# algbio/SBWT

Hardware: AMD Instinct MI355X
Metric: k-mers/sec (whole node), plain-matrix k=30 streaming search (higher is better)
Workload: dtype u64

## Files before the change

sbwt_amd/csrc/sbwt_device.h:

```cpp
#pragma once
#include <stdint.h>

#define SBWT_MEGA_SHIFT 31
#define SBWT_GROUP_BASES 32

#ifndef SBWT_FUSED_SORT_DEFAULT
#define SBWT_FUSED_SORT_DEFAULT 3632
#endif
struct SbwtIndexView {
    const uint4 *blocks;
    const longlong2 *ptab;
    const unsigned long long *mega;
    long long n_nodes;
    long long n_pos;
    long long C[4];
    int k;
    int p_dev;
    int n_mega;
    int has_ssup;
    int probe_len;
    const uint4 *stab;
    int p_sparse;
    unsigned n_sb;
    const unsigned *col, *pos;
// ... 52 lines not shown
#define SBWT_SP_OVERFLOW (1ull << 62)
#define SBWT_SP_UNIQ 0x80000000u
#define SBWT_SP_MAX_DEPTH 31
#define SBWT_SP_HASH 0x9E3779B97F4A7C15ull
static __host__ __device__ inline unsigned long long sp2_hash(unsigned origin, unsigned long long key2) {
    unsigned long long h = (key2 ^ ((unsigned long long)origin << 17)) * SBWT_SP_HASH;
    h ^= h >> 31;
    return (h + origin) * 0xD6E8FEB86659FD93ull;
}
#define SBWT_SP2_USED 0x80000000u
#define SBWT_SP2_OVERFLOW 0x80000000u
static __host__ __device__ inline unsigned long long sbwt_pf_hash(unsigned long long key) { return key * SBWT_SP_HASH; }
static __host__ __device__ inline unsigned sbwt_pf_bits(unsigned long long h) { return (unsigned)(h >> 24) ^ (unsigned)(h >> 41); }

struct SbwtWorkHeader {
    unsigned long long ticket;
    int status;
    int rg_sample;
    unsigned long long n_stream;
    unsigned long long n_search;
    unsigned long long n_lf;
    unsigned long long n_tab_hit;
    unsigned long long n_ext;
    unsigned long long n_bridge;
    unsigned long long u_bad;
    long long u_read0, u_len, u_out0, u_stride;
    unsigned long long n_deferred;
    unsigned long long ticket2;
    unsigned long long n_pieces;
    unsigned long long pad[15];
    unsigned long long rg_long;
    unsigned long long n_ftick;
    unsigned long long ftick_over;
    unsigned long long pad2[5];
    unsigned long long hint;
};
#define SBWT_WS_CLEAR_BYTES (sizeof(SbwtWorkHeader) - 8)

#define SBWT_PIECE 1024
struct SbwtPieceTab {
    uint4 *pairs = nullptr;
    uint4 *outs = nullptr;
    long long cap = 0;
    int piece = SBWT_PIECE;
};
static_assert(sizeof(SbwtWorkHeader) == 320, "workspace header is 320 bytes");
struct SbwtTickTab {
    uint4 *tick = nullptr;
    unsigned *tick_read = nullptr;
    unsigned *defer_bits = nullptr;
    long long cap = 0;
};
#define SBWT_HINT_MAGIC 0x5B377A00u
#define SBWT_HINT_RATIO 12
#define SBWT_HINT_CALLS 2

void sbwt_launch_encode(const char *d_bases, long long total_bases, uint4 *d_packed, SbwtWorkHeader *ws,
                        hipStream_t stream);
void sbwt_launch_search(const SbwtIndexView &ix, const uint4 *d_packed, const long long *d_read_off,
                        const long long *d_out_off, long long *d_out, long long n_reads, SbwtWorkHeader *ws,
                        int streaming, hipStream_t stream, int variant, long long total_groups, void *d_sort_scratch,
                        long long sort_scratch_bytes, int sort_key_bits, SbwtPieceTab pt);
void sbwt_launch_search_fused(const SbwtIndexView &ix, const char *d_bases, long long total_bases, uint4 *d_packed,
                              const long long *d_read_off, const long long *d_out_off, long long *d_out, long long n_reads,
                              SbwtWorkHeader *ws, int streaming, hipStream_t stream, unsigned *d_defer,
                              hipEvent_t ev_begin, hipEvent_t ev_end, SbwtPieceTab pt, int ragged_ok, SbwtTickTab tt = SbwtTickTab());
void sbwt_launch_encode_chained(const char *d_bases, long long total_bases, uint4 *d_packed, SbwtWorkHeader *ws,
// ... 64 lines not shown
```

sbwt_amd/csrc/sbwt_kernels_common.h:

```cpp
#pragma once
#include <hip/hip_runtime.h>
#include <cstdio>
#include <cstdlib>
#include "sbwt_device.h"

typedef unsigned long long u64;
typedef long long i64;

#define SBWT_ERR_NOT_SINGLETON (-7)
#define SBWT_ERR_STALLED (-10)

__device__ __forceinline__ unsigned dna_code(unsigned b) { return ((b >> 1) & 3u) ^ ((b >> 2) & 1u); }
__device__ __forceinline__ bool is_ACGT(unsigned b) { return b == 'A' || b == 'C' || b == 'G' || b == 'T'; }
__device__ __forceinline__ u64 quad_bits(const uint4 &q) { return (u64)q.x | ((u64)q.y << 32); }
__device__ __forceinline__ u64 low_mask(int n) { return (1ull << n) - 1ull; }

__device__ __forceinline__ unsigned uniform32(unsigned v) { return (unsigned)__builtin_amdgcn_readfirstlane((int)v); }
__device__ __forceinline__ u64 uniform64(u64 v) {
    return (u64)(unsigned)__builtin_amdgcn_readfirstlane((int)(unsigned)v) |
           ((u64)(unsigned)__builtin_amdgcn_readfirstlane((int)(unsigned)(v >> 32)) << 32);
}

typedef unsigned u32x4 __attribute__((ext_vector_type(4)));
#ifdef SBWT_PLAIN_STORES
#define SBWT_NT_STORE(v, p) (*(p) = (v))
#else
#define SBWT_NT_STORE(v, p) __builtin_nontemporal_store(v, p)
#endif
__device__ __forceinline__ void st_stream(i64 *p, i64 v) { SBWT_NT_STORE(v, p); }
typedef i64 i64x2_a8 __attribute__((ext_vector_type(2), aligned(8)));
typedef unsigned u32x2_a4 __attribute__((ext_vector_type(2), aligned(4)));
__device__ __forceinline__ void st_stream2(i64 *p, i64 a, i64 b) {
    i64x2_a8 v = {a, b};
    SBWT_NT_STORE(v, reinterpret_cast<i64x2_a8 *>(p));
}
typedef int i32x2_a4 __attribute__((ext_vector_type(2), aligned(4)));
__device__ __forceinline__ void st_res(i64 *out, i64 at, i64 v, int o32) {
    if (o32) SBWT_NT_STORE((int)v, reinterpret_cast<int *>(out) + at);
    else st_stream(out + at, v);
}
__device__ __forceinline__ void st_res2(i64 *out, i64 at, i64 a, i64 b, int o32) {
    if (o32) {
        i32x2_a4 v = {(int)a, (int)b};
        SBWT_NT_STORE(v, reinterpret_cast<i32x2_a4 *>(reinterpret_cast<int *>(out) + at));
    } else {
        st_stream2(out + at, a, b);
    }
}
__device__ __forceinline__ uint4 ld_stream(const uint4 *p) {
    u32x4 v = __builtin_nontemporal_load(reinterpret_cast<const u32x4 *>(p));
    return make_uint4(v.x, v.y, v.z, v.w);
}

template <bool MEGA>
__device__ __forceinline__ u64 quad_rank(const SbwtIndexView &ix, const uint4 &q, i64 pos, int c) {
    u64 v = (u64)q.z + (u64)__popcll(quad_bits(q) & low_mask((int)(pos & 63)));
    if (MEGA) v += ix.mega[(i64)c * ix.n_mega + (pos >> SBWT_MEGA_SHIFT)];
    return v;
}

template <bool MEGA>
__device__ __forceinline__ u64 block_count(const SbwtIndexView &ix, i64 blk, int c, uint4 *q) {
    *q = ix.blocks[(blk << 2) + c];
    u64 v = (u64)q->z;
    if (MEGA) v += ix.mega[(i64)c * ix.n_mega + (blk >> (SBWT_MEGA_SHIFT - 6))];
    return v;
}

template <bool MEGA>
__device__ __forceinline__ i64 select_in_row(const SbwtIndexView &ix, int c, i64 target_i, i64 row_ones) {
    const u64 target = (u64)target_i;
    const i64 n_blocks = ix.n_nodes / 64 + 1;
    i64 g = row_ones > 0 ? (i64)((double)(target_i - ix.C[c]) / (double)row_ones * (double)n_blocks) : 0;
    if (g < 0) g = 0;
    if (g > n_blocks - 1) g = n_blocks - 1;
    uint4 q;
    i64 lo, hi;
    if (block_count<MEGA>(ix, g, c, &q) <= target) {
        lo = g;
        i64 step = 1;
        hi = g + step;
// ... 122 lines not shown
```

sbwt_amd/csrc/sbwt_search_fused.hip:

```cpp
#include "sbwt_kernels_common.h"

#define F_IDLE 0
#define F_INIT 2
#define F_STEP 3
#define F_DEAD 4
#define F_EXT 7
#define F_TRANS 8
#define F_POS 9
#define F_BRIDGE 10
#define F_CMP 11
#define F_PLAN 12
#define FE_NONE 0
#define FE_EMIT1 1
#define FE_FAIL 2
#define FE_END 3
#define FE_PRES 4
#define FE_ANCH 5
#ifndef FZ_ANCHORS
#define FZ_ANCHORS 3
#endif
#ifndef FZ_ALIGNS
#define FZ_ALIGNS 7
#endif
#define CF_S1 1u
// ... 106 lines not shown
#define FZ_PLAN_SUM(q, val) do { } while (0)
#endif

#ifdef SBWT_TIMELINE
__device__ unsigned long long g_fz_tl[8];
__device__ unsigned long long g_fz_tl_hist[1024];
extern "C" int sbwtgpu_debug_timeline(unsigned long long *out, int reset) {
    if (out && (hipMemcpyFromSymbol(out, HIP_SYMBOL(g_fz_tl), sizeof(g_fz_tl)) != hipSuccess ||
                hipMemcpyFromSymbol(out + 8, HIP_SYMBOL(g_fz_tl_hist), sizeof(g_fz_tl_hist)) != hipSuccess)) return -1;
    if (reset) {
        static unsigned long long z[1024];
        unsigned long long t0[8] = {~0ull, ~0ull, 0, 0, 0, 0, 0, 0};
        if (hipMemcpyToSymbol(HIP_SYMBOL(g_fz_tl), t0, sizeof(t0)) != hipSuccess ||
            hipMemcpyToSymbol(HIP_SYMBOL(g_fz_tl_hist), z, sizeof(g_fz_tl_hist)) != hipSuccess) return -1;
    }
    return 0;
}
#endif

__device__ __forceinline__ u64 fz_encode32(const unsigned w[8], const unsigned tm[8], unsigned &bad) {
    u64 codes = 0;
#pragma unroll
    for (int d = 0; d < 8; d++) {
        const unsigned x = w[d];
        const unsigned t = ((x >> 1) & 0x03030303u) ^ ((x >> 2) & 0x01010101u);
        const unsigned c8 = (t * 0x01041040u) >> 24;
        const unsigned letters = __builtin_amdgcn_perm(0x54474341u, 0x54474341u, t);
        bad |= (letters ^ x) & tm[d];
        codes |= (u64)c8 << (8 * d);
    }
    return codes;
}

#ifdef FZ_SORT_WG5
#define FZ_SLOTS 256
#define FZ_RING 256
#define FZ_SORT_WGS 5
#else
#define FZ_SLOTS 320
#define FZ_RING 512
#define FZ_SORT_WGS 4
#endif
template <bool WIDE, bool O32, bool BIG = false, bool UNI = false, bool SORT = false, bool TAB = false>
__global__ void __launch_bounds__(256, SORT ? FZ_SORT_WGS : 5) k_search_fused(SbwtIndexView ix, const unsigned char *__restrict__ bases,
                                                          i64 total_bases, i64 *__restrict__ out, i64 n_reads,
                                                          SbwtWorkHeader *ws, unsigned *__restrict__ defer_list,
                                                          const i64 *__restrict__ read_off, const i64 *__restrict__ out_off,
                                                          SbwtTickTab tt) {
    static_assert(!SORT || (!WIDE && !BIG), "lanes sorted by state: k <= 31, fewer than 2^31 columns (so far)");
    __shared__ u64 pool_codes[SBWT_FUSED_MAXG][SORT ? 128 : 256];
    constexpr int NSLOT = SORT ? FZ_SLOTS : 256;
    __shared__ u64 cur_codes[SBWT_FUSED_MAXG][NSLOT];
    __shared__ unsigned seg_src[FZ_NSEG][NSLOT];
    __shared__ unsigned char seg_at[FZ_NSEG][NSLOT];
    __shared__ unsigned st_w[SORT ? 4 : 1][SORT ? FZ_SLOTS : 1];
    __shared__ unsigned short q_ring[SORT ? 2 : 1][SORT ? FZ_RING : 1];
    __shared__ unsigned q_ctl[8];
    const int fmode = sbwt_fused_mode(ws, ix.k);
    if (fmode == 0) return;
    const int P_batch = sbwt_fused_pieces(ws, ix.k);
    if (UNI != (fmode == 1 && P_batch == 1 && !(ix.debug & 128))) return;
    const bool ragged = !UNI && fmode == 2;
    static_assert(!TAB || !UNI, "the ticket table's instantiation is a general one");
    const bool table = TAB && fmode == 3 && tt.tick != nullptr;
    if (TAB != (fmode == 3)) return;
    if (!WIDE && !BIG && ix.fused_sort > 0) {
        const bool sorted_call = (ix.fused_sort & 4096) ||
                                 (ws->hint == (unsigned long long)(SBWT_HINT_MAGIC | (unsigned)SBWT_HINT_CALLS) && (UNI || TAB || P_batch == 1));
        if (SORT != sorted_call) return;
    } else if (SORT) return;
    const int tid = threadIdx.x, lane = tid & 63, wbase = tid & ~63;
    const bool follower_wave = SORT && __builtin_amdgcn_readfirstlane(tid) >= 128;
    int slot = SORT ? (follower_wave ? -1 : tid) : tid;
    if (SORT) {
        if (tid < 8) q_ctl[tid] = (tid == 2) ? (unsigned)(FZ_SLOTS - 128) : 0u;
        for (int q = tid; q < (SORT ? FZ_RING : 0); q += 256) {
            q_ring[0][SORT ? q : 0] = q < FZ_SLOTS - 128 ? (unsigned short)(128 + q + 1) : (unsigned short)0;
            q_ring[SORT ? 1 : 0][SORT ? q : 0] = 0;
        }
        for (int q = 128 + tid; q < (SORT ? FZ_SLOTS : 0); q += 256) st_w[SORT ? 2 : 0][SORT ? q : 0] = 0u;
        __syncthreads();
    }
#define FZ_LDS32(p) (*(__attribute__((address_space(3))) volatile unsigned *)(p))
#define FZ_LDS16(p) (*(__attribute__((address_space(3))) volatile unsigned short *)(p))
    auto ring_push = [&](const u64 mask, const int ring, const int s) {
        unsigned base = 0;
        if (lane == 0) base = __hip_atomic_fetch_add(&q_ctl[2 + ring], (unsigned)__popcll(mask), __ATOMIC_RELAXED, __HIP_MEMORY_SCOPE_WORKGROUP);
        base = uniform32(base);
        if ((mask >> lane) & 1ull) {
            const unsigned at = (base + (unsigned)__popcll(mask & low_mask(lane))) & (unsigned)(FZ_RING - 1);
            asm volatile("s_waitcnt lgkmcnt(0)" ::: "memory");
            FZ_LDS16(&q_ring[SORT ? ring : 0][SORT ? at : 0]) = (unsigned short)(s + 1);
        }
    };
    const int k = ix.k, p = ix.p_dev, L0 = ix.probe_len, ps = ix.p_sparse;
    const int P = (UNI || table) ? 1 : P_batch, kpp = SBWT_FUSED_MAXLEN - k + 1;
    const bool varlen = ragged || table || P > 1;
    const i64 n_tickets = table ? (i64)ws->n_ftick : n_reads * P;
    const int ulen = (ragged || table) ? SBWT_FUSED_MAXLEN : (int)ws->u_len, m = ulen - k + 1, G = varlen ? SBWT_FUSED_MAXG : ((ulen + 31) >> 5);
    const i64 u_read0 = ws->u_read0, u_out0 = ws->u_out0, u_stride = ws->u_stride;
    const bool pfon = ix.pfil && ix.p_filter == L0 && L0 > p;
// ... 61 lines not shown
#include "sbwt_search_fused_loop.inc"
    }

    FZ_HIST_FLUSH();
#ifdef SBWT_TIMELINE
    if (lane == 0) {
        const u64 tl_exit = wall_clock64(), t0 = g_fz_tl[0];
        atomicMin(&g_fz_tl[1], tl_drain); atomicMax(&g_fz_tl[2], tl_drain); atomicMax(&g_fz_tl[3], tl_exit);
        atomicAdd(&g_fz_tl[4], 1ull); atomicAdd(&g_fz_tl[5], tl_exit - tl_drain); atomicAdd(&g_fz_tl[6], tl_exit - tl_start);
        atomicAdd(&g_fz_tl[7], (unsigned long long)tl_n);
        const u64 bk = (tl_exit - t0) / 1000ull;
        atomicAdd(&g_fz_tl_hist[bk < 1023 ? bk : 1023], 1ull);
    }
#endif
    {
        u64 e = c_ext & 0xFFFFFu, eb = c_ext >> 20;
#pragma unroll
        for (int off = 32; off > 0; off >>= 1) { e += __shfl_down(e, off); eb += __shfl_down(eb, off); }
        if (lane == 0) { if (e) atomicAdd(&ws->n_ext, e); if (eb) atomicAdd(&ws->n_bridge, eb); }
    }
#if defined(SBWT_SORT_COUNTERS) && !defined(SBWT_STATS)
    if (SORT && lane == 0) {
        atomicAdd(&ws->pad[follower_wave ? 13 : 11], (unsigned long long)c_iter);
        atomicAdd(&ws->pad[follower_wave ? 14 : 12], c_busy);
        atomicAdd(&ws->pad[9], (unsigned long long)c_lists);
        atomicAdd(&ws->pad[10], (unsigned long long)c_part);
    }
#endif
    if (lane == 0) {
        if (c_stream) atomicAdd(&ws->n_stream, (u64)c_stream);
        if (c_search) atomicAdd(&ws->n_search, (u64)c_search);
        if (c_lf) atomicAdd(&ws->n_lf, (u64)c_lf);
        if (c_tab) atomicAdd(&ws->n_tab_hit, (u64)c_tab);
    }
}

__global__ void __launch_bounds__(256) k_fused_tickets(const i64 *__restrict__ read_off, const i64 *__restrict__ out_off, i64 n_reads,
                                                       SbwtWorkHeader *ws, int k, SbwtTickTab tt) {
    if (!sbwt_fused_wants_table(ws, k)) return;
    const int lane = threadIdx.x & 63;
    const int kpp = SBWT_FUSED_MAXLEN - k + 1;
    const i64 stride = (i64)gridDim.x * 256;
    for (i64 r0 = (i64)blockIdx.x * 256 + (threadIdx.x & ~63); r0 < n_reads; r0 += stride) {
        const i64 r = r0 + lane;
        const bool valid = r < n_reads;
        const i64 P0 = valid ? read_off[r] : 0, len = valid ? read_off[r + 1] - P0 : 0, ob = valid ? out_off[r] : 0;
        const i64 m = len - k + 1;
        const u64 np = m > 0 ? (u64)((m + kpp - 1) / kpp) : 0ull;
        u64 incl = np;
#pragma unroll
        for (int o = 1; o < 64; o <<= 1) { const u64 v = __shfl_up(incl, o); if (lane >= o) incl += v; }
        const u64 total = __shfl(incl, 63);
        if (total == 0) continue;
        u64 base = 0;
        if (lane == 0) base = atomicAdd(&ws->n_ftick, (unsigned long long)total);
        base = uniform64(base);
        if (base + total > (u64)tt.cap) {
            if (lane == 0) ws->ftick_over = 1ull;
            continue;
        }
        const u64 first = base + incl - np;
        auto entry = [&](i64 rr, i64 p0, i64 ln, i64 o0, u64 t0, u64 j) {
            const i64 b = p0 + (i64)j * kpp, left = ln - (i64)j * kpp;
            const unsigned nb = (unsigned)(left > SBWT_FUSED_MAXLEN ? SBWT_FUSED_MAXLEN : left);
            const i64 o = o0 + (i64)j * kpp;
            tt.tick[t0 + j] = make_uint4((unsigned)b, ((unsigned)((u64)b >> 32) & 0xFFFFu) | (nb << 16), (unsigned)o, (unsigned)((u64)o >> 32));
            tt.tick_read[t0 + j] = (unsigned)rr;
        };
        for (u64 j = 0; j < np && j < 4; j++) entry(r, P0, len, ob, first, j);
        u64 big = __ballot(np > 4);
        while (big) {
            const int src = __ffsll((i64)big) - 1;
            big &= big - 1;
            const i64 rr = __shfl(r, src), p0 = __shfl(P0, src), ln = __shfl(len, src), o0 = __shfl(ob, src);
            const u64 t0 = __shfl(first, src), nn = __shfl(np, src);
            for (u64 j = 4 + (u64)lane; j < nn; j += 64) entry(rr, p0, ln, o0, t0, j);
        }
    }
}

__global__ void k_fused_hint(SbwtWorkHeader *ws, int k) {
    if (threadIdx.x != 0 || sbwt_fused_mode(ws, k) == 0) return;
    const unsigned long long ext = ws->n_ext, walks = ws->n_search, prev = ws->hint;
    const bool fits = walks > 0 && ext >= (unsigned long long)SBWT_HINT_RATIO * walks;
    const unsigned run = ((prev & ~0xFFull) == (unsigned long long)SBWT_HINT_MAGIC) ? (unsigned)(prev & 0xFFull) : 0u;
    ws->hint = (unsigned long long)(SBWT_HINT_MAGIC | (fits ? (run < SBWT_HINT_CALLS ? run + 1u : (unsigned)SBWT_HINT_CALLS) : 0u));
}

__global__ void __launch_bounds__(256) k_check_uniform2(const i64 *__restrict__ read_off, const i64 *__restrict__ out_off,
                                                        i64 n_reads, SbwtWorkHeader *ws, int k, SbwtPieceTab pt,
                                                        int rg_enable) {
    const i64 t = (i64)blockIdx.x * 256 + threadIdx.x;
    const i64 len = read_off[1] - read_off[0], stride = (n_reads > 1) ? out_off[1] - out_off[0] : 0;
    if (t == 0) { ws->u_read0 = read_off[0]; ws->u_len = len; ws->u_out0 = out_off[0]; ws->u_stride = stride; }
    const bool valid = t < n_reads;
    const i64 mylen = valid ? read_off[t + 1] - read_off[t] : 0;
    fused_sample_of_wave(t, mylen, valid, n_reads, rg_enable, k, ws);
    piece_zones_of_wave(t, mylen, valid, k, ws, pt);
    if (!valid) return;
    const bool bad = (mylen != len) || (t + 1 < n_reads && out_off[t + 1] - out_off[t] != stride);
    if (__ballot(bad) != 0 && (threadIdx.x & 63) == 0) ws->u_bad = 1ull;
}

void sbwt_launch_search_fused(const SbwtIndexView &ix, const char *d_bases, long long total_bases, uint4 *d_packed,
                              const long long *d_read_off, const long long *d_out_off, long long *d_out, long long n_reads,
                              SbwtWorkHeader *ws, int streaming, hipStream_t stream, unsigned *d_defer,
                              hipEvent_t ev_begin, hipEvent_t ev_end, SbwtPieceTab pt, int ragged_ok, SbwtTickTab tt) {
    if (n_reads <= 0) return;
    hipLaunchKernelGGL(k_check_uniform2, dim3(grid_for(n_reads)), dim3(256), 0, stream, d_read_off, d_out_off, (i64)n_reads, ws,
                       ix.k, pt, ragged_ok);
    if (tt.tick && n_reads < ((i64)1 << 32)) {
        const i64 wantt = (n_reads + 255) / 256;
        hipLaunchKernelGGL(k_fused_tickets, dim3((unsigned)(wantt < 1024 ? wantt : 1024)), dim3(256), 0, stream, d_read_off, d_out_off,
                           (i64)n_reads, ws, ix.k, tt);
    }
    const i64 want_r = (n_reads + 255) / 256, want_t = tt.tick ? (total_bases / SBWT_FUSED_MAXLEN + 255) / 256 : 0;
    const i64 want = want_r > want_t ? want_r : want_t;
    unsigned cap = 1280u;
    if (ix.debug >> 8) cap = (unsigned)(ix.debug >> 8);
    else if (total_bases < 8000000ll) cap = 256u;
    else if (total_bases < 20000000ll) cap = 384u;
    else if (total_bases < 60000000ll) cap = 512u;
    else if (total_bases < 110000000ll) cap = 640u;
    else if (total_bases < 170000000ll) cap = 768u;
    else if (total_bases < 250000000ll) cap = 896u;
    else if (total_bases < 500000000ll) cap = 1024u;
    const bool sorted = !ix.big && !(ix.n_nodes >= ((i64)1 << 31) - 64) && !((ix.stab2 != nullptr && ix.p_sparse < ix.k) || (ix.debug & 64)) && ix.fused_sort > 0;
    const unsigned cap_s = cap > 256u * FZ_SORT_WGS ? 256u * FZ_SORT_WGS : cap;
    const unsigned g = (unsigned)(want < (i64)cap ? want : (i64)cap), g_s = (unsigned)(want < (i64)cap_s ? want : (i64)cap_s);
    if (ev_begin) (void)hipEventRecord(ev_begin, stream);
    const bool wide = (ix.stab2 != nullptr && ix.p_sparse < ix.k) || (ix.debug & 64);
#define FZ_LAUNCH1(W, O, B, U) hipLaunchKernelGGL((k_search_fused<W, O, B, U>), dim3(g), dim3(256), 0, stream, ix, \
                                           reinterpret_cast<const unsigned char *>(d_bases), (i64)total_bases, d_out, (i64)n_reads, ws, d_defer, \
                                           d_read_off, d_out_off, tt)
#define FZ_LAUNCH(W, O, B) do { FZ_LAUNCH1(W, O, B, true); FZ_LAUNCH1(W, O, B, false); \
                                if (tt.tick) hipLaunchKernelGGL((k_search_fused<W, O, B, false, false, true>), dim3(g), dim3(256), 0, stream, ix, \
                                           reinterpret_cast<const unsigned char *>(d_bases), (i64)total_bases, d_out, (i64)n_reads, ws, d_defer, \
                                           d_read_off, d_out_off, tt); } while (0)
#define FZ_LAUNCH_S(O) do { hipLaunchKernelGGL((k_search_fused<false, O, false, true, true>), dim3(g_s), dim3(256), 0, stream, ix, \
                                           reinterpret_cast<const unsigned char *>(d_bases), (i64)total_bases, d_out, (i64)n_reads, ws, d_defer, \
                                           d_read_off, d_out_off, tt); \
                            hipLaunchKernelGGL((k_search_fused<false, O, false, false, true>), dim3(g_s), dim3(256), 0, stream, ix, \
                                           reinterpret_cast<const unsigned char *>(d_bases), (i64)total_bases, d_out, (i64)n_reads, ws, d_defer, \
                                           d_read_off, d_out_off, tt); \
                            if (tt.tick) hipLaunchKernelGGL((k_search_fused<false, O, false, false, true, true>), dim3(g_s), dim3(256), 0, stream, ix, \
                                           reinterpret_cast<const unsigned char *>(d_bases), (i64)total_bases, d_out, (i64)n_reads, ws, d_defer, \
                                           d_read_off, d_out_off, tt); } while (0)
    const bool big = ix.big || ix.n_nodes >= ((i64)1 << 31) - 64;
    if (big) { if (wide) FZ_LAUNCH(true, false, true); else FZ_LAUNCH(false, false, true); }
    else if (wide) { if (ix.out32) FZ_LAUNCH(true, true, false); else FZ_LAUNCH(true, false, false); }
    else {
        if (ix.out32) FZ_LAUNCH(false, true, false); else FZ_LAUNCH(false, false, false);
        if (sorted) { if (ix.out32) FZ_LAUNCH_S(true); else FZ_LAUNCH_S(false); }
    }
#undef FZ_LAUNCH_S
#undef FZ_LAUNCH
#undef FZ_LAUNCH1
    if (ev_end) (void)hipEventRecord(ev_end, stream);
    if (sorted) hipLaunchKernelGGL(k_fused_hint, dim3(1), dim3(64), 0, stream, ws, ix.k);
    sbwt_launch_encode_chained(d_bases, total_bases, d_packed, ws, d_defer, d_read_off, ix.k, stream);
    sbwt_launch_piece_bounds_tt(d_packed, d_read_off, d_out_off, ix.k, ws, pt, 1, stream, tt.defer_bits);
    sbwt_launch_search_chained(ix, d_packed, d_read_off, d_out_off, d_out, n_reads, ws, streaming, stream, d_defer, pt);
}
```

sbwt_amd/csrc/sbwt_search_fused_loop.inc:

```
    for (;;) {
#ifdef SBWT_STATS
        int pl_kind = -1, oc_kind = -1, cert_n = 0;
#endif
        bool force = false;
        bool w31 = false;
        auto plan_walk = [&](bool force, const bool w31) {
            int s0 = i, nwk = (ps > 0) ? 1 : 0;
            bool win31 = false;
            if (w31 && (fl & CF_MISS_MASK) < 2u * CF_MISS && b >= i && b <= i + k - 1) {
                const int ws = b < i + k - ps ? b : i + k - ps;
                if (ws > i) { win31 = true; force = false; s0 = ws; }
            }
            if ((fl & CF_MISS_MASK) >= 2u * CF_MISS) force = true;
            bool hinted = false;
            if (!force && pfon && !(b >= i && b <= i + k - 1) && bnext >= i && bnext <= i + k - 1) { b = blo = bnext; bnext = -1; hinted = true; }
            if (win31) {
                nwk = 1;
                fl |= CF_WIN31;
            } else if (!force && L0 > 0 && b >= i && b <= i + k - 1) {
                const int lo = blo > i ? blo : i;
                if (lo < b && anch_ok && CF_ANC_LEFT(fl) > 0 && b + 1 != CF_ANC_TRIED(fl) && b + 1 <= mend - 1) {
                    s0 = b + 1;
                    nwk = 1;
                    fl |= CF_ANCH;
// ... 94 lines not shown
                            rlen = read_off[tb] - rstart;
                        } else {
                            rstart = u_read0 + tr * ulen;
                            rlen = tr < n_reads ? ulen : 0;
                        }
                        toolong = rlen > sbwt_fused_limit(P, k);
                        const i64 pstart = rstart + (i64)pc * kpp, plen = rlen - (i64)pc * kpp;
                        woff = (i64)uniform64((u64)rstart);
                        if (table) {
                            i64 lo = (i64)pool_next + lane < n_tickets ? rstart : (i64)0x7FFFFFFFFFFFFFFFll;
#pragma unroll
                            for (int o = 32; o > 0; o >>= 1) { const i64 v = __shfl_xor(lo, o); lo = v < lo ? v : lo; }
                            woff = lo == (i64)0x7FFFFFFFFFFFFFFFll ? 0 : lo;
                        }
                        const i64 rel = pstart - woff;
                        vrel = (rel < 0 || rel > 0xFFFF0000ll) ? 0xFFFF0000u : (unsigned)rel;
                        len_l = toolong ? SBWT_FUSED_MAXLEN + 1 : plen <= 0 ? 0 : plen > SBWT_FUSED_MAXLEN ? SBWT_FUSED_MAXLEN : (int)plen;
                        pool_len = len_l | (pc << 16);
                    }
                    const int len_e = len_l > SBWT_FUSED_MAXLEN ? SBWT_FUSED_MAXLEN : len_l;
                    i64 remain = total_bases - woff;
                    if (remain < 0) remain = 0;
                    if (remain > 0xFFFFFFF0ll) remain = 0xFFFFFFF0ll;
                    const unsigned char *p0 = bases + woff;
                    const unsigned delta = (unsigned)((uintptr_t)p0 & 3u);
                    __amdgpu_buffer_rsrc_t rs = __builtin_amdgcn_make_buffer_rsrc(
                        const_cast<unsigned char *>(p0 - delta), (short)0, (int)(((unsigned)remain + delta + 3u) & ~3u), 0x00020000);
                    const unsigned vo = delta + vrel;
                    unsigned bad = 0;
#pragma unroll
                    for (int g = 0; g < SBWT_FUSED_MAXG; g++) {
                        if (g < G) {
                            const unsigned o = vo + 32u * (unsigned)g, oa = o & ~3u, sh = o & 3u;
                            const fz_u32x4 x0 = __builtin_amdgcn_raw_buffer_load_b128(rs, (int)oa, 0, 0);
                            const fz_u32x4 x1 = __builtin_amdgcn_raw_buffer_load_b128(rs, (int)oa + 16, 0, 0);
                            const unsigned x2 = __builtin_amdgcn_raw_buffer_load_b32(rs, (int)oa + 32, 0, 0);
                            const unsigned raw[9] = {x0.x, x0.y, x0.z, x0.w, x1.x, x1.y, x1.z, x1.w, x2};
                            unsigned w[8], tm[8];
#pragma unroll
                            for (int d = 0; d < 8; d++) {
                                w[d] = __builtin_amdgcn_alignbyte(raw[d + 1], raw[d], sh);
                                const int nb = len_e - 32 * g - 4 * d;
                                tm[d] = nb >= 4 ? 0xFFFFFFFFu : nb <= 0 ? 0u : ((1u << (8 * nb)) - 1u);
                            }
                            pool_codes[g][wbase + lane] = fz_encode32(w, tm, bad);
                        }
                    }
                    const bool isbad = (bad != 0 || toolong) && (i64)(pool_next + (u64)lane) < n_tickets;
                    pool_bad = __ballot(isbad);
                    const u64 defer_m = __ballot(isbad && (!toolong || pc == 0));
                    if (defer_m) {
                        unsigned long long at = 0;
                        if (lane == 0) at = atomicAdd(&ws->n_deferred, (unsigned long long)__popcll(defer_m));
                        at = uniform64(at);
                        if ((defer_m >> lane) & 1ull) {
                            const unsigned dr = table ? tt.tick_read[pool_next + (u64)lane]
                                : (unsigned)(P == 1 ? (pool_next + (u64)lane) : P == 2 ? ((pool_next + (u64)lane) >> 1) : (pool_next + (u64)lane) / 3ull);
                            defer_list[at + (u64)__popcll(defer_m & low_mask(lane))] = dr;
                            if (table) atomicOr(&tt.defer_bits[dr >> 5], 1u << (dr & 31u));
                        }
                    }
                } else {
                    drained = true;
                    if (SORT && lane == 0) (void)__hip_atomic_fetch_add(&q_ctl[5], 1u, __ATOMIC_RELAXED, __HIP_MEMORY_SCOPE_WORKGROUP);
#ifdef SBWT_TIMELINE
                    tl_drain = wall_clock64();
#endif
                    pool_end = pool_next;
                }
// ... 268 lines not shown
#pragma unroll
            for (int u = 0; u < FP; u++) {
                fL[u] = -1; fe[u] = 0; fa[u] = 0; fob[u] = 0; w0[u] = w1[u] = 0;
                if (fm == 0) continue;
                const int L = __ffsll((i64)fm) - 1;
                fm &= fm - 1;
                const int pdL = __builtin_amdgcn_readlane(pend, L);
                const int ns = (pdL >> 16) & 15, a = pdL & 0xFF, e = (pdL >> 8) & 0xFF;
                const bool direct = (pdL >> 22) & 1;
                fL[u] = L;
                fa[u] = a;
#ifdef SBWT_SORT_COUNTERS
                if (SORT) { c_lists = uniform32(c_lists + 1u); if (!((pdL >> 23) & 1)) c_part = uniform32(c_part + 1u); }
#endif
                {
                    const unsigned prL = (unsigned)__builtin_amdgcn_readlane((int)pend_rd, L);
                    if (SORT) fsl[u] = (int)prL;
                    const i64 rdu = SORT ? (i64)uniform32(st_w[0][SORT ? (int)prL : 0]) : (i64)prL;
                    if (!UNI && table) {
                        const uint4 te = tt.tick[rdu];
                        fob[u] = (i64)uniform64(((u64)te.w << 32) | (u64)te.z);
                    } else
                    fob[u] = (ragged ? out_off[rdu] : u_out0 + rdu * u_stride) + (UNI ? 0 : (i64)(((pdL >> 20) & 3) * kpp));
                }
                slow = slow || direct || (e - a > 128);
                if (direct) continue;
                fe[u] = e;
                const int j0 = a + 2 * lane, j1 = j0 + 1;
                unsigned c0s, c1s;
                int c0a, c1a;
                seg_of(SORT ? fsl[u] : wbase + L, ns, j0, c0s, c0a, c1s, c1a);
                const unsigned p0 = (j0 < e && c0s != 0xFFFFFFFFu) ? c0s + (unsigned)(j0 - c0a) : col_minus1;
                const unsigned p1 = (j1 < e && c1s != 0xFFFFFFFFu) ? c1s + (unsigned)(j1 - c1a) : col_minus1;
                w0[u] = (int)ix.col[p0];
                w1[u] = (int)ix.col[p1];
            }
            return slow;
        };
        auto flush_store = [&](const bool slow) {
#pragma unroll
            for (int u = 0; u < FP; u++) asm volatile("" : "+v"(w0[u]), "+v"(w1[u]));
            if (!(ix.debug & 1)) {
#pragma unroll
                for (int u = 0; u < FP; u++) {
                    const int fj = fa[u] + 2 * lane;
                    const i64 r0 = BIG ? (w0[u] == -1 ? -1ll : (i64)(unsigned)w0[u]) : (i64)w0[u];
                    const i64 r1 = BIG ? (w1[u] == -1 ? -1ll : (i64)(unsigned)w1[u]) : (i64)w1[u];
                    if (fj + 1 < fe[u]) st_res2(out, fob[u] + fj, r0, r1, O32);
                    else if (fj < fe[u]) st_res(out, fob[u] + fj, r0, O32);
                }
            }
            if (slow) {
#pragma unroll
                for (int u = 0; u < FP; u++) {
                    if (fL[u] < 0) continue;
                    const int L = fL[u], pdL = __builtin_amdgcn_readlane(pend, L);
                    const int ns = (pdL >> 16) & 15, a = pdL & 0xFF, e = (pdL >> 8) & 0xFF;
                    for (int base = ((pdL >> 22) & 1) ? a : a + 128; base < e; base += 128) {
                        const int j0 = base + 2 * lane, j1 = j0 + 1;
                        unsigned c0s, c1s;
                        int c0a, c1a;
                        seg_of(SORT ? fsl[u] : wbase + L, ns, j0, c0s, c0a, c1s, c1a);
                        const unsigned p0 = (j0 < e && is_run(c0s)) ? c0s + (unsigned)(j0 - c0a) : col_minus1;
                        const unsigned p1 = (j1 < e && is_run(c1s)) ? c1s + (unsigned)(j1 - c1a) : col_minus1;
                        const int y0 = (int)ix.col[p0], y1 = (int)ix.col[p1];
                        const int q0 = is_run(c0s) ? y0 : ((c0s == 0xFFFFFFFFu) ? -1 : (int)(c0s & 0x7FFFFFFFu));
                        const int q1 = is_run(c1s) ? y1 : ((c1s == 0xFFFFFFFFu) ? -1 : (int)(c1s & 0x7FFFFFFFu));
                        const i64 r0 = BIG ? (q0 == -1 ? -1ll : (i64)(unsigned)q0) : (i64)q0;
                        const i64 r1 = BIG ? (q1 == -1 ? -1ll : (i64)(unsigned)q1) : (i64)q1;
                        if (!(ix.debug & 1)) {
                            if (j1 < e) st_res2(out, fob[u] + j0, r0, r1, O32);
                            else if (j0 < e) st_res(out, fob[u] + j0, r0, O32);
                        }
                    }
                }
            }
        };
        uint4 v1, v2;
        if (fm_pend) {
            u64 fm = fm_pend;
            bool lr = flush_issue(fm);
            v1 = *a1;
            v2 = *a2;
            flush_store(lr);
            while (fm) {
                lr = flush_issue(fm);
                flush_store(lr);
            }
            if (SORT) {
                const u64 fin = fm_pend & __ballot((pend >> 23) & 1);
                if (fin) {
                    if (lane == 0) (void)__hip_atomic_fetch_sub(&q_ctl[4], (unsigned)__popcll(fin), __ATOMIC_RELAXED, __HIP_MEMORY_SCOPE_WORKGROUP);
                    if (isP) {
                        const int ps_ = (int)pend_rd;
                        if ((fin >> lane) & 1ull) st_w[SORT ? 2 : 0][SORT ? ps_ : 0] = 0u;
                        ring_push(fin, 0, ps_);
                        FZ_SORT_STAT(10, __popcll(fin));
                    }
                }
            }
        } else {
            v1 = *a1;
            v2 = *a2;
        }

// ... 619 lines not shown
```

sbwt_amd/csrc/sbwtgpu_capi.cpp:

```cpp
#include <hip/hip_runtime.h>

#include <dlfcn.h>
#include <cstdarg>
#include <chrono>
#include <cstdio>
#include <cstdlib>
#include <algorithm>
#include <mutex>
#include <cstddef>
#include <cstring>
#include <new>
#include <vector>
#include <thread>

#include "../../include/sbwtgpu.h"
#include "sbwt_device.h"
#include "sbwt_ms.h"

namespace {

thread_local char g_err[512] = "";

int fail(int code, const char *fmt, ...) {
    va_list ap;
// ... 989 lines not shown
                             void *d_ws, int64_t ws_bytes, void *stream, int streaming) {
    int rc = search_dev_check(idx, total_bases, n_reads, d_ws, ws_bytes, streaming);
    if (rc != SBWTGPU_OK) return rc;
    if (n_reads == 0) return SBWTGPU_OK;
    {
        int variant = g_variant_override >= 0 ? g_variant_override : tuning_variant();
        if (variant < 0) variant = idx->h.has_path ? auto_variant(idx->h) : 2;
        const int eff_streaming = (!streaming && internal_streaming_ok(idx->h)) ? 2 : streaming;
        const bool big_image = idx->h.big_layout && idx->h.has_path && !t_out32 &&
                               ((idx->h.stab_pos && idx->h.p_sparse == idx->h.k) || (idx->h.n_sb2 > 0 && idx->h.k > idx->h.p_sparse));
        const bool path_kernel = idx->h.has_path && eff_streaming &&
                                 ((idx->h.n_nodes < ((int64_t)1 << 31) - 128 && !idx->h.big_layout) || big_image) && n_reads < ((int64_t)1 << 31) &&
                                 total_bases / SBWT_GROUP_BASES + 2 < ((int64_t)1 << 31) - 4;
        if (variant == 5 && path_kernel && g_sort_reads <= 0 && !(g_debug & 16)) {
            if (!d_read_off || !d_out_off) return fail(SBWTGPU_ERR_INVALID_ARG, "NULL device pointer");
            if (total_bases > 0 && !d_bases) return fail(SBWTGPU_ERR_INVALID_ARG, "NULL device pointer");
            DeviceGuard guard(idx->device);
            hipStream_t st = static_cast<hipStream_t>(stream);
            SbwtWorkHeader *ws = static_cast<SbwtWorkHeader *>(d_ws);
            HIP_TRY(hipMemsetAsync(ws, 0, SBWT_WS_CLEAR_BYTES, st));
            if (g_poison) {
                int64_t ends[2] = {0, 0};
                HIP_TRY(hipMemcpyAsync(&ends[0], d_out_off, 8, hipMemcpyDeviceToHost, st));
                HIP_TRY(hipMemcpyAsync(&ends[1], d_out_off + n_reads, 8, hipMemcpyDeviceToHost, st));
                HIP_TRY(hipStreamSynchronize(st));
                if (ends[1] > ends[0]) {
                    const size_t vb = t_out32 ? 4 : 8;
                    HIP_TRY(hipMemsetAsync(reinterpret_cast<char *>(d_out) + (size_t)ends[0] * vb, 0xA5, (size_t)(ends[1] - ends[0]) * vb, st));
                }
            }
            uint4 *packed = reinterpret_cast<uint4 *>(static_cast<char *>(d_ws) + sizeof(SbwtWorkHeader));
            unsigned *defer = reinterpret_cast<unsigned *>(static_cast<char *>(d_ws) + align256(ws_packed_bytes(total_bases)));
            const SbwtTickTab tt_of_call = ws_tick_tab(d_ws, total_bases);
            HIP_TRY(hipMemsetAsync(tt_of_call.defer_bits, 0, (size_t)(total_bases / 256 + 64), st));
            SbwtTickTab tt_for_launch = tt_of_call;
            if (!(g_fused_table && g_fused_ragged && n_reads <= total_bases / 32)) { tt_for_launch.tick = nullptr; tt_for_launch.tick_read = nullptr; }
            hipEvent_t e0 = nullptr, e1 = nullptr;
            if (g_kernel_events) {
                const int slot = (int)(g_ev_count % EV_RING);
                if (slot >= g_ev_made) {
                    HIP_TRY(hipEventCreate(&g_ev[slot][0]));
                    HIP_TRY(hipEventCreate(&g_ev[slot][1]));
                    g_ev_made = slot + 1;
                }
                e0 = g_ev[slot][0]; e1 = g_ev[slot][1];
                g_ev_count++;
            }
            sbwt_launch_search_fused(idx->view(), d_bases, total_bases, packed, reinterpret_cast<const long long *>(d_read_off),
                                     reinterpret_cast<const long long *>(d_out_off), reinterpret_cast<long long *>(d_out), n_reads,
                                     ws, eff_streaming, st, defer, e0, e1, ws_piece_tab(d_ws, total_bases),
                                     ((g_fused_ragged && n_reads <= total_bases / 32) ? 1 : 0) |
                                         ((g_fused_pieces > 0 ? g_fused_pieces : 3) << 8),
                                     tt_for_launch);
            hipError_t e = hipGetLastError();
            if (e != hipSuccess) return fail(SBWTGPU_ERR_HIP, "kernel launch: %s", hipGetErrorString(e));
            return SBWTGPU_OK;
        }
    }
    rc = sbwtgpu_encode_bases_dev(idx, d_bases, total_bases, d_ws, ws_bytes, stream);
    if (rc != SBWTGPU_OK) return rc;
    return sbwtgpu_search_encoded_dev(idx, total_bases, d_read_off, n_reads, d_out, d_out_off, d_ws, ws_bytes,
                                      streaming, stream);
}

int sbwtgpu_streaming_search_dev(const sbwtgpu_index *idx, const char *d_bases, int64_t total_bases,
                                 const int64_t *d_read_off, int64_t n_reads, int64_t *d_out,
                                 const int64_t *d_out_off, void *d_ws, int64_t ws_bytes, void *stream) {
// ... 1315 lines not shown
```

Measured before the change: 265.8 billion.

## Fold fused hint into last wave and defer-bit clear into check kernel

```diff
diff --git a/sbwt_amd/csrc/sbwt_device.h b/sbwt_amd/csrc/sbwt_device.h
--- a/sbwt_amd/csrc/sbwt_device.h
+++ b/sbwt_amd/csrc/sbwt_device.h
@@ -108,7 +108,9 @@
     unsigned long long rg_long;
     unsigned long long n_ftick;
     unsigned long long ftick_over;
-    unsigned long long pad2[5];
+    unsigned long long hint_in;
+    unsigned long long fused_done;
+    unsigned long long pad2[3];
     unsigned long long hint;
 };
 #define SBWT_WS_CLEAR_BYTES (sizeof(SbwtWorkHeader) - 8)
diff --git a/sbwt_amd/csrc/sbwt_kernels_common.h b/sbwt_amd/csrc/sbwt_kernels_common.h
--- a/sbwt_amd/csrc/sbwt_kernels_common.h
+++ b/sbwt_amd/csrc/sbwt_kernels_common.h
@@ -47,6 +47,50 @@
         st_stream2(out + at, a, b);
     }
 }
+#ifndef SBWT_RESULT_STORE
+#define SBWT_RESULT_STORE 0
+#endif
+#if SBWT_RESULT_STORE != 0
+#define SBWT_RESULT_AUX (SBWT_RESULT_STORE == 2 ? 17 : 16)
+typedef unsigned u32x2 __attribute__((ext_vector_type(2)));
+__device__ __forceinline__ __amdgpu_buffer_rsrc_t st_row_rsrc(i64 *out, i64 row, int o32) {
+    char *base = reinterpret_cast<char *>(out) + (o32 ? row * 4 : row * 8);
+    return __builtin_amdgcn_make_buffer_rsrc(reinterpret_cast<char *>((uintptr_t)uniform64((u64)(uintptr_t)base)), (short)0, 4096, 0x00020000);
+}
+#endif
+__device__ __forceinline__ void st_row(i64 *out, i64 row, int j, i64 v, int o32) {
+#if SBWT_RESULT_STORE != 0
+    const __amdgpu_buffer_rsrc_t rs = st_row_rsrc(out, row, o32);
+    if (o32) __builtin_amdgcn_raw_buffer_store_b32((unsigned)v, rs, j * 4, 0, SBWT_RESULT_AUX);
+    else {
+        const u32x2 w = {(unsigned)v, (unsigned)((u64)v >> 32)};
+        __builtin_amdgcn_raw_buffer_store_b64(w, rs, j * 8, 0, SBWT_RESULT_AUX);
+    }
+#else
+    st_res(out, row + j, v, o32);
+#endif
+}
+__device__ __forceinline__ void st_row2(i64 *out, i64 row, int j, i64 a, i64 b, int o32) {
+#if SBWT_RESULT_STORE != 0
+    const __amdgpu_buffer_rsrc_t rs = st_row_rsrc(out, row, o32);
+    if (o32) {
+        const u32x2 w = {(unsigned)a, (unsigned)b};
+        __builtin_amdgcn_raw_buffer_store_b64(w, rs, j * 4, 0, SBWT_RESULT_AUX);
+    } else {
+        const u32x4 w = {(unsigned)a, (unsigned)((u64)a >> 32), (unsigned)b, (unsigned)((u64)b >> 32)};
+        __builtin_amdgcn_raw_buffer_store_b128(w, rs, j * 8, 0, SBWT_RESULT_AUX);
+    }
+#else
+    st_res2(out, row + j, a, b, o32);
+#endif
+}
+#ifdef SBWT_STREAM_LOADS
+#define SBWT_COL_LOAD(p) __builtin_nontemporal_load(p)
+#define SBWT_BASE_LOAD_AUX 2
+#else
+#define SBWT_COL_LOAD(p) (*(p))
+#define SBWT_BASE_LOAD_AUX 0
+#endif
 __device__ __forceinline__ uint4 ld_stream(const uint4 *p) {
     u32x4 v = __builtin_nontemporal_load(reinterpret_cast<const u32x4 *>(p));
     return make_uint4(v.x, v.y, v.z, v.w);
diff --git a/sbwt_amd/csrc/sbwt_search_fused.hip b/sbwt_amd/csrc/sbwt_search_fused.hip
--- a/sbwt_amd/csrc/sbwt_search_fused.hip
+++ b/sbwt_amd/csrc/sbwt_search_fused.hip
@@ -162,6 +162,14 @@
     return codes;
 }
 
+__device__ __forceinline__ void fused_write_hint(SbwtWorkHeader *ws) {
+    const unsigned long long ext = __hip_atomic_load(&ws->n_ext, __ATOMIC_RELAXED, __HIP_MEMORY_SCOPE_AGENT),
+                             walks = __hip_atomic_load(&ws->n_search, __ATOMIC_RELAXED, __HIP_MEMORY_SCOPE_AGENT), prev = ws->hint_in;
+    const bool fits = walks > 0 && ext >= (unsigned long long)SBWT_HINT_RATIO * walks;
+    const unsigned run = ((prev & ~0xFFull) == (unsigned long long)SBWT_HINT_MAGIC) ? (unsigned)(prev & 0xFFull) : 0u;
+    ws->hint = (unsigned long long)(SBWT_HINT_MAGIC | (fits ? (run < SBWT_HINT_CALLS ? run + 1u : (unsigned)SBWT_HINT_CALLS) : 0u));
+}
+
 #ifdef FZ_SORT_WG5
 #define FZ_SLOTS 256
 #define FZ_RING 256
@@ -196,7 +204,7 @@
     if (TAB != (fmode == 3)) return;
     if (!WIDE && !BIG && ix.fused_sort > 0) {
         const bool sorted_call = (ix.fused_sort & 4096) ||
-                                 (ws->hint == (unsigned long long)(SBWT_HINT_MAGIC | (unsigned)SBWT_HINT_CALLS) && (UNI || TAB || P_batch == 1));
+                                 (ws->hint_in == (unsigned long long)(SBWT_HINT_MAGIC | (unsigned)SBWT_HINT_CALLS) && (UNI || TAB || P_batch == 1));
         if (SORT != sorted_call) return;
     } else if (SORT) return;
     const int tid = threadIdx.x, lane = tid & 63, wbase = tid & ~63;
@@ -324,6 +332,11 @@
         if (c_search) atomicAdd(&ws->n_search, (u64)c_search);
         if (c_lf) atomicAdd(&ws->n_lf, (u64)c_lf);
         if (c_tab) atomicAdd(&ws->n_tab_hit, (u64)c_tab);
+        if (!WIDE && !BIG && ix.fused_sort > 0) {
+            asm volatile("s_waitcnt vmcnt(0)" ::: "memory");
+            const u64 done = atomicAdd(&ws->fused_done, 1ull);
+            if (done + 1ull == (u64)gridDim.x * (u64)(blockDim.x >> 6)) fused_write_hint(ws);
+        }
     }
 }
 
@@ -371,20 +384,13 @@
     }
 }
 
-__global__ void k_fused_hint(SbwtWorkHeader *ws, int k) {
-    if (threadIdx.x != 0 || sbwt_fused_mode(ws, k) == 0) return;
-    const unsigned long long ext = ws->n_ext, walks = ws->n_search, prev = ws->hint;
-    const bool fits = walks > 0 && ext >= (unsigned long long)SBWT_HINT_RATIO * walks;
-    const unsigned run = ((prev & ~0xFFull) == (unsigned long long)SBWT_HINT_MAGIC) ? (unsigned)(prev & 0xFFull) : 0u;
-    ws->hint = (unsigned long long)(SBWT_HINT_MAGIC | (fits ? (run < SBWT_HINT_CALLS ? run + 1u : (unsigned)SBWT_HINT_CALLS) : 0u));
-}
-
 __global__ void __launch_bounds__(256) k_check_uniform2(const i64 *__restrict__ read_off, const i64 *__restrict__ out_off,
                                                         i64 n_reads, SbwtWorkHeader *ws, int k, SbwtPieceTab pt,
-                                                        int rg_enable) {
+                                                        int rg_enable, unsigned *__restrict__ defer_bits) {
     const i64 t = (i64)blockIdx.x * 256 + threadIdx.x;
+    if (defer_bits && t < (n_reads + 31) / 32) defer_bits[t] = 0u;
     const i64 len = read_off[1] - read_off[0], stride = (n_reads > 1) ? out_off[1] - out_off[0] : 0;
-    if (t == 0) { ws->u_read0 = read_off[0]; ws->u_len = len; ws->u_out0 = out_off[0]; ws->u_stride = stride; }
+    if (t == 0) { ws->u_read0 = read_off[0]; ws->u_len = len; ws->u_out0 = out_off[0]; ws->u_stride = stride; ws->hint_in = ws->hint; }
     const bool valid = t < n_reads;
     const i64 mylen = valid ? read_off[t + 1] - read_off[t] : 0;
     fused_sample_of_wave(t, mylen, valid, n_reads, rg_enable, k, ws);
@@ -400,7 +406,7 @@
                               hipEvent_t ev_begin, hipEvent_t ev_end, SbwtPieceTab pt, int ragged_ok, SbwtTickTab tt) {
     if (n_reads <= 0) return;
     hipLaunchKernelGGL(k_check_uniform2, dim3(grid_for(n_reads)), dim3(256), 0, stream, d_read_off, d_out_off, (i64)n_reads, ws,
-                       ix.k, pt, ragged_ok);
+                       ix.k, pt, ragged_ok, tt.tick ? tt.defer_bits : nullptr);
     if (tt.tick && n_reads < ((i64)1 << 32)) {
         const i64 wantt = (n_reads + 255) / 256;
         hipLaunchKernelGGL(k_fused_tickets, dim3((unsigned)(wantt < 1024 ? wantt : 1024)), dim3(256), 0, stream, d_read_off, d_out_off,
@@ -449,7 +455,6 @@
 #undef FZ_LAUNCH
 #undef FZ_LAUNCH1
     if (ev_end) (void)hipEventRecord(ev_end, stream);
-    if (sorted) hipLaunchKernelGGL(k_fused_hint, dim3(1), dim3(64), 0, stream, ws, ix.k);
     sbwt_launch_encode_chained(d_bases, total_bases, d_packed, ws, d_defer, d_read_off, ix.k, stream);
     sbwt_launch_piece_bounds_tt(d_packed, d_read_off, d_out_off, ix.k, ws, pt, 1, stream, tt.defer_bits);
     sbwt_launch_search_chained(ix, d_packed, d_read_off, d_out_off, d_out, n_reads, ws, streaming, stream, d_defer, pt);
diff --git a/sbwt_amd/csrc/sbwt_search_fused_loop.inc b/sbwt_amd/csrc/sbwt_search_fused_loop.inc
--- a/sbwt_amd/csrc/sbwt_search_fused_loop.inc
+++ b/sbwt_amd/csrc/sbwt_search_fused_loop.inc
@@ -150,9 +150,9 @@
                     for (int g = 0; g < SBWT_FUSED_MAXG; g++) {
                         if (g < G) {
                             const unsigned o = vo + 32u * (unsigned)g, oa = o & ~3u, sh = o & 3u;
-                            const fz_u32x4 x0 = __builtin_amdgcn_raw_buffer_load_b128(rs, (int)oa, 0, 0);
-                            const fz_u32x4 x1 = __builtin_amdgcn_raw_buffer_load_b128(rs, (int)oa + 16, 0, 0);
-                            const unsigned x2 = __builtin_amdgcn_raw_buffer_load_b32(rs, (int)oa + 32, 0, 0);
+                            const fz_u32x4 x0 = __builtin_amdgcn_raw_buffer_load_b128(rs, (int)oa, 0, SBWT_BASE_LOAD_AUX);
+                            const fz_u32x4 x1 = __builtin_amdgcn_raw_buffer_load_b128(rs, (int)oa + 16, 0, SBWT_BASE_LOAD_AUX);
+                            const unsigned x2 = __builtin_amdgcn_raw_buffer_load_b32(rs, (int)oa + 32, 0, SBWT_BASE_LOAD_AUX);
                             const unsigned raw[9] = {x0.x, x0.y, x0.z, x0.w, x1.x, x1.y, x1.z, x1.w, x2};
                             unsigned w[8], tm[8];
 #pragma unroll
@@ -487,8 +487,8 @@
                 seg_of(SORT ? fsl[u] : wbase + L, ns, j0, c0s, c0a, c1s, c1a);
                 const unsigned p0 = (j0 < e && c0s != 0xFFFFFFFFu) ? c0s + (unsigned)(j0 - c0a) : col_minus1;
                 const unsigned p1 = (j1 < e && c1s != 0xFFFFFFFFu) ? c1s + (unsigned)(j1 - c1a) : col_minus1;
-                w0[u] = (int)ix.col[p0];
-                w1[u] = (int)ix.col[p1];
+                w0[u] = (int)SBWT_COL_LOAD(&ix.col[p0]);
+                w1[u] = (int)SBWT_COL_LOAD(&ix.col[p1]);
             }
             return slow;
         };
@@ -501,8 +501,8 @@
                     const int fj = fa[u] + 2 * lane;
                     const i64 r0 = BIG ? (w0[u] == -1 ? -1ll : (i64)(unsigned)w0[u]) : (i64)w0[u];
                     const i64 r1 = BIG ? (w1[u] == -1 ? -1ll : (i64)(unsigned)w1[u]) : (i64)w1[u];
-                    if (fj + 1 < fe[u]) st_res2(out, fob[u] + fj, r0, r1, O32);
-                    else if (fj < fe[u]) st_res(out, fob[u] + fj, r0, O32);
+                    if (fj + 1 < fe[u]) st_row2(out, fob[u], fj, r0, r1, O32);
+                    else if (fj < fe[u]) st_row(out, fob[u], fj, r0, O32);
                 }
             }
             if (slow) {
@@ -518,14 +518,14 @@
                         seg_of(SORT ? fsl[u] : wbase + L, ns, j0, c0s, c0a, c1s, c1a);
                         const unsigned p0 = (j0 < e && is_run(c0s)) ? c0s + (unsigned)(j0 - c0a) : col_minus1;
                         const unsigned p1 = (j1 < e && is_run(c1s)) ? c1s + (unsigned)(j1 - c1a) : col_minus1;
-                        const int y0 = (int)ix.col[p0], y1 = (int)ix.col[p1];
+                        const int y0 = (int)SBWT_COL_LOAD(&ix.col[p0]), y1 = (int)SBWT_COL_LOAD(&ix.col[p1]);
                         const int q0 = is_run(c0s) ? y0 : ((c0s == 0xFFFFFFFFu) ? -1 : (int)(c0s & 0x7FFFFFFFu));
                         const int q1 = is_run(c1s) ? y1 : ((c1s == 0xFFFFFFFFu) ? -1 : (int)(c1s & 0x7FFFFFFFu));
                         const i64 r0 = BIG ? (q0 == -1 ? -1ll : (i64)(unsigned)q0) : (i64)q0;
                         const i64 r1 = BIG ? (q1 == -1 ? -1ll : (i64)(unsigned)q1) : (i64)q1;
                         if (!(ix.debug & 1)) {
-                            if (j1 < e) st_res2(out, fob[u] + j0, r0, r1, O32);
-                            else if (j0 < e) st_res(out, fob[u] + j0, r0, O32);
+                            if (j1 < e) st_row2(out, fob[u], j0, r0, r1, O32);
+                            else if (j0 < e) st_row(out, fob[u], j0, r0, O32);
                         }
                     }
                 }
diff --git a/sbwt_amd/csrc/sbwtgpu_capi.cpp b/sbwt_amd/csrc/sbwtgpu_capi.cpp
--- a/sbwt_amd/csrc/sbwtgpu_capi.cpp
+++ b/sbwt_amd/csrc/sbwtgpu_capi.cpp
@@ -1045,7 +1045,6 @@
             uint4 *packed = reinterpret_cast<uint4 *>(static_cast<char *>(d_ws) + sizeof(SbwtWorkHeader));
             unsigned *defer = reinterpret_cast<unsigned *>(static_cast<char *>(d_ws) + align256(ws_packed_bytes(total_bases)));
             const SbwtTickTab tt_of_call = ws_tick_tab(d_ws, total_bases);
-            HIP_TRY(hipMemsetAsync(tt_of_call.defer_bits, 0, (size_t)(total_bases / 256 + 64), st));
             SbwtTickTab tt_for_launch = tt_of_call;
             if (!(g_fused_table && g_fused_ragged && n_reads <= total_bases / 32)) { tt_for_launch.tick = nullptr; tt_for_launch.tick_read = nullptr; }
             hipEvent_t e0 = nullptr, e1 = nullptr;
```

Result: no change. 266.5 billion (median of 6 runs) (+0.3%).
